# smolGura/fish-tts

Measured on AMD Instinct MI355X. Metric: semantic tokens/sec, higher is better.
Workload: dtype bf16; 1 GPU; openaudio-s1-mini shapes (BASELINE configs[1]): batch=1 per GPU, 48-token prompt, 215 frames (10 s), top-p sampling, hipGraph-captured frame step, + DAC codec decode; prompt_len=48, parallelism=replica x1, frame_engine=3

## Files before the change

fish-tts_amd/csrc/engine.hip:

```cpp
#include "engine.h"
#include "ar_kernels.h"
#include "frame_engine.h"
#include "wide_kernels.h"
#include "codec_kernels.h"

#include <math.h>

#include <algorithm>
#include <mutex>
#include <stdarg.h>
#include <stdio.h>
#include <stdlib.h>
#include <string.h>

using namespace ft;

static std::string g_create_err;
static void eng_release(ft_ctx* ctx);

ft_status ft_fail(ft_ctx* ctx, ft_status code, const std::string& msg) {
    if (ctx) ctx->err = msg; else g_create_err = msg;
    return code;
}

// ... 2051 lines not shown
            if (it->first & (1 << 28)) { hipGraphExecDestroy(it->second); it = ctx->graphs.erase(it); } else ++it;
        }
        eng_release(ctx);
        snprintf(buf, sizeof buf, "launch path: the frame engine was turned off after %d hand-off time-outs (last in phase %u)",
                 ctx->eng_strikes, w[ENG_CTL_WHERE]);
        ctx->eng_why = buf;
    }
    fprintf(stderr, "fish_tts_amd: frame engine: a hand-off timed out (phase %u, strike %d of %d): the frames are redone on the "
            "launch path%s\n", w[ENG_CTL_WHERE], ctx->eng_strikes, ENG_MAX_STRIKES,
            ctx->eng_strikes >= ENG_MAX_STRIKES ? "; the engine stays off for this context" : "");
    return FT_OK;
}
static bool eng_in_use(const ft_ctx* ctx) { return (ctx->eng_on || ctx->eng_fast_on) && !ctx->eng_suspended; }

extern "C" ft_status ft_ar_engine_state(ft_ctx* ctx, int32_t* flags, int32_t* aborted, int32_t* where) {
    FT_TRY(ar_ready(ctx));
    if (flags) *flags = (ctx->eng_on ? 1 : 0) | (ctx->eng_fast_on ? 2 : 0);
    if (aborted) *aborted = ctx->eng_strikes;
    if (where) *where = ctx->eng_last_where;
    return FT_OK;
}

extern "C" const char* ft_ar_frame_path(const ft_ctx* ctx) {
    if (!ctx) return "";
    ft_ctx* c = const_cast<ft_ctx*>(ctx);
    c->path_str = ctx->eng_why + (ctx->wide_ok
                                      ? "; lock-step batches of >= 5 rows: MFMA launches with fused row operations (five per layer)"
                                      : "; lock-step batches: multi-row GEMV launches");
    return c->path_str.c_str();
}

extern "C" ft_status ft_test_engine_fault(ft_ctx* ctx, int32_t which, int32_t wg, int32_t skip) {
    FT_TRY(ar_ready(ctx));
    if (!ctx->eng_ctl || !(which == 0 ? ctx->eng_on : ctx->eng_fast_on)) return ft_fail(ctx, FT_ERR_STATE, "ft_test_engine_fault: the frame engine is off");
    if (wg < 0 || wg >= ctx->eng_nb || skip < 0) return ft_fail(ctx, FT_ERR_ARG, "ft_test_engine_fault: bad workgroup or skip count");
    const unsigned v[2] = {(which == 0 ? 0u : ENG_FAULT_FAST) + 1u + (unsigned)wg, (unsigned)skip};
    static_assert(ENG_CTL_FAULT_SKIP == ENG_CTL_FAULT + 1, "the two words are written by one copy");
    FT_HIP(ctx, hipStreamSynchronize(ctx->stream));
    FT_HIP(ctx, hipMemcpy(ctx->eng_ctl + ENG_CTL_FAULT, v, sizeof v, hipMemcpyHostToDevice));
    return FT_OK;
}

extern "C" ft_status ft_test_ar_attn_plan(ft_ctx* ctx, int32_t* nsplit, int32_t* xl, int32_t* n_slots) {
    FT_TRY(ar_ready(ctx));
    if (nsplit) *nsplit = ctx->nsplit;
    if (xl) *xl = ctx->eng_on && ctx->eng_xl ? 1 : 0;
    if (n_slots) *n_slots = ctx->n_slots;
    return FT_OK;
}

namespace {
extern "C" ft_status ft_test_ar_trace_arm(ft_ctx* ctx, int32_t first, int32_t count) {
    FT_TRY(ar_ready(ctx));
    if (first < 0 || count < 0) return ft_fail(ctx, FT_ERR_ARG, "ft_test_ar_trace_arm: bad range");
    if (ctx->c.max_batch == 1 && eng_in_use(ctx))
        return ft_fail(ctx, FT_ERR_STATE, "ft_test_ar_trace_arm: this context's frames run on the frame engine");
    ArTrace& t = ctx->tstore;
    t.recs.clear();
    t.first = first; t.count = count; t.armed = true; t.failed = false; t.kind = 0;
    return FT_OK;
}
extern "C" int32_t ft_test_ar_trace_count(ft_ctx* ctx, int32_t* info) {
    if (!ctx || !ctx->has_ar) return -1;
    const ArTrace& t = ctx->tstore;
    if (info) { info[0] = t.kind; info[1] = t.m0; info[2] = t.M; info[3] = t.armed ? 1 : 0; info[4] = (int32_t)t.begin.size(); }
    return t.failed ? -1 : (int32_t)t.recs.size();
}
extern "C" ft_status ft_test_ar_trace_launch(ft_ctx* ctx, int32_t i, char* name, int32_t cap, int32_t* info) {
    if (!ctx || !ctx->has_ar || !name || cap < 1 || !info) return FT_ERR_ARG;
// ... 1148 lines not shown
```

fish-tts_amd/csrc/frame_engine.h:

```cpp
#pragma once
#include "ar_kernels.h"

namespace ft {

constexpr int ENG_NB = 256;
constexpr int ENG_WAVES = 8;
constexpr int ENG_THREADS = ENG_WAVES * 64;
constexpr int ENG_CW = 4;
constexpr int ENG_GW = 4;

template <int D_, int H_, int HKV_, int HDIM_, int F_>
struct EngSlowShape {
    static constexpr int D = D_, H = H_, HKV = HKV_, HDIM = HDIM_, F = F_;
    static constexpr int HD = H * HDIM, QKVN = (H + 2 * HKV) * HDIM, G = H / HKV;
    static constexpr int NTD = D / 512, NTA = HD / 512, NTF = F / 512;
    static constexpr int SQ = (QKVN / ENG_NB + ENG_CW - 1) / ENG_CW, SF = (F / ENG_NB + ENG_CW - 1) / ENG_CW, SO = (D / ENG_NB + ENG_CW - 1) / ENG_CW;
    static constexpr bool PK3 = F % 384 == 0 && (F / ENG_NB) % 3 == 0;
    static_assert(D % 512 == 0 && HD % 512 == 0 && F % 512 == 0, "weight rows are read as whole 16-byte pieces by 64 lanes");
    static_assert(QKVN % (4 * ENG_NB) == 0 && D % (4 * ENG_NB) == 0 && F % (4 * ENG_NB) == 0, "whole 16-byte granule groups per workgroup");
    static_assert(H % HKV == 0 && HDIM % 8 == 0 && HDIM <= 128, "grouped-query attention, 16-byte K/V pieces");
};
template <int D_, int H_, int HKV_, int HDIM_, int F_, int V_>
struct EngFastShape {
    static constexpr int D = D_, H = H_, HKV = HKV_, HDIM = HDIM_, F = F_, V = V_;
    static constexpr int HD = H * HDIM, QKVN = (H + 2 * HKV) * HDIM, KVW = HKV * HDIM;
    static constexpr int NTD = D / 512, NTA = HD / 512, NTF = F / 512;
    static constexpr int SQ = (QKVN / ENG_NB + ENG_CW - 1) / ENG_CW, SF = (F / ENG_NB + ENG_CW - 1) / ENG_CW, SO = (D / ENG_NB + ENG_CW - 1) / ENG_CW;
    static constexpr bool PK3 = F % 384 == 0 && (F / ENG_NB) % 3 == 0;
    static constexpr int RESF = (NTD <= 2 && F / ENG_NB == 12) ? 2 : 0;
    static constexpr int RESL = RESF ? 4 : 0;
    static_assert(D % 512 == 0 && HD % 512 == 0 && F % 512 == 0 && V == 1024 && HD == D, "fast widths");
    static_assert(QKVN % (4 * ENG_NB) == 0 && D % (4 * ENG_NB) == 0 && F % (4 * ENG_NB) == 0 && V % (4 * ENG_NB) == 0, "whole granule groups per workgroup");
};
typedef EngSlowShape<1024, 16, 8, 128, 3072> EngSlowS1;
typedef EngFastShape<1024, 16, 8, 64, 3072, 1024> EngFastS1;
constexpr int ENG_EPOCH_STEP = 64;
constexpr unsigned long long ENG_TIMEOUT_TICKS = 20000000ull;

typedef __attribute__((address_space(1))) unsigned eng_gu32;
typedef __attribute__((address_space(1))) unsigned long long eng_gu64;
#define ENG_RLX __ATOMIC_RELAXED, __HIP_MEMORY_SCOPE_AGENT

enum { ENG_CTL_EPOCH = 0, ENG_CTL_ABORT = 1, ENG_CTL_EXIT = 2, ENG_CTL_WHERE = 3, ENG_CTL_ARRIVED = 4, ENG_CTL_FAULT = 5, ENG_CTL_FAULT_SKIP = 6,
       ENG_CTL_XCD = 16, ENG_CTL_WORDS = 32 };
constexpr unsigned ENG_FAULT_FAST = 0x10000u;
__device__ __forceinline__ bool eng_fault_here(unsigned* ctl, unsigned base, int b) {
    const unsigned f = __hip_atomic_load((__attribute__((address_space(1))) unsigned*)(ctl + ENG_CTL_FAULT), __ATOMIC_RELAXED, __HIP_MEMORY_SCOPE_AGENT);
    if (f != base + 1u + (unsigned)b) return false;
    const unsigned skip = __hip_atomic_load((__attribute__((address_space(1))) unsigned*)(ctl + ENG_CTL_FAULT_SKIP), __ATOMIC_RELAXED, __HIP_MEMORY_SCOPE_AGENT);
    if (skip > 0u) {
        __hip_atomic_store((__attribute__((address_space(1))) unsigned*)(ctl + ENG_CTL_FAULT_SKIP), skip - 1u, __ATOMIC_RELAXED, __HIP_MEMORY_SCOPE_AGENT);
        return false;
    }
    __hip_atomic_store((__attribute__((address_space(1))) unsigned*)(ctl + ENG_CTL_FAULT), 0u, __ATOMIC_RELAXED, __HIP_MEMORY_SCOPE_AGENT);
    return true;
}

struct EngLayer {
    const bf16_t *wqkv, *bqkv, *attn_norm, *qn, *kn, *wo, *bo, *ffn_norm, *w13, *w2;
    bf16_t *kc, *vc;
};

__device__ __forceinline__ void eng_barrier() {
    __builtin_amdgcn_fence(__ATOMIC_RELEASE, "workgroup", "local");
    __builtin_amdgcn_s_barrier();
    __builtin_amdgcn_fence(__ATOMIC_ACQUIRE, "workgroup", "local");
}

typedef const __attribute__((address_space(1))) U4* eng_gU4;
template <bool NT> __device__ __forceinline__ U4 eng_ldg16(const void* p) {
    if constexpr (NT) return __builtin_nontemporal_load((eng_gU4)p);
    else return *(eng_gU4)p;
}
__device__ __forceinline__ float eng_ldg_bf16(const bf16_t* p, size_t i) {
    return bf16_bits_to_f32(((const __attribute__((address_space(1))) bf16_t*)p)[i]);
}
typedef const __attribute__((address_space(4))) unsigned long long* eng_c64;
__device__ __forceinline__ EngLayer eng_layer(const EngLayer* table, int i) {
    static_assert(sizeof(EngLayer) == 12 * sizeof(unsigned long long), "EngLayer is twelve pointers");
    eng_c64 q = (eng_c64)(unsigned long long)(table + i);
    EngLayer l;
    l.wqkv = (const bf16_t*)q[0]; l.bqkv = (const bf16_t*)q[1]; l.attn_norm = (const bf16_t*)q[2]; l.qn = (const bf16_t*)q[3];
    l.kn = (const bf16_t*)q[4]; l.wo = (const bf16_t*)q[5]; l.bo = (const bf16_t*)q[6]; l.ffn_norm = (const bf16_t*)q[7];
    l.w13 = (const bf16_t*)q[8]; l.w2 = (const bf16_t*)q[9]; l.kc = (bf16_t*)q[10]; l.vc = (bf16_t*)q[11];
    return l;
}

__device__ __forceinline__ unsigned eng_tag16(unsigned e) { return (e & 0x7fffu) | 0x8000u; }
// ... 76 lines not shown
    EngSpin sp{ctl, dead, 0, 0, where};
    unsigned long long n_full = 0, t_first = 0;
    for (int p0 = gw; p0 < npiece; p0 += 3 * ngw) {
        const int c0 = p0;
        const int c1 = p0 + ngw < npiece ? p0 + ngw : c0;
        const int c2 = p0 + 2 * ngw < npiece ? p0 + 2 * ngw : c0;
        const int i0 = c0 * 256 + lane * 4 < n ? c0 * 256 + lane * 4 : c0 * 256;
        const int i1 = c1 * 256 + lane * 4 < n ? c1 * 256 + lane * 4 : c1 * 256;
        const int i2 = c2 * 256 + lane * 4 < n ? c2 * 256 + lane * 4 : c2 * 256;
        const int o0 = lay.off(u0 + i0), o1 = lay.off(u0 + i1), o2 = lay.off(u0 + i2);
        U4 a, b, c;
        for (;;) {
            if (c1 == c0) { eng_ld1_sc1<FL>(g + o0, a); b = a; c = a; }
            else eng_ld3_sc1<FL>(g + o0, g + o1, g + o2, a, b, c);
            const bool oa = eng_tags_ok(a, tag), ob = eng_tags_ok(b, tag), oc = eng_tags_ok(c, tag);
            if (dbg && n_full == 0) t_first = eng_rt();
            ++n_full;
            if (__all(oa && ob && oc)) break;
            if (sp.give_up(lane)) return;
        }
        if (c0 * 256 + lane * 4 < n) eng_unpack_to_lds(dst + dmap(i0), a);
        if (c1 != c0 && c1 * 256 + lane * 4 < n) eng_unpack_to_lds(dst + dmap(i1), b);
        if (c2 != c0 && c2 * 256 + lane * 4 < n) eng_unpack_to_lds(dst + dmap(i2), c);
    }
    if (dbg && lane == 0) { dbg[0] = t_first; dbg[1] = n_full; dbg[2] = 0; }
}

struct EngRelay {
    int on;
    int rank, nr;
    long delta;
};

__device__ __forceinline__ void eng_register(unsigned* ctl, int nb, int* r, int* dead) {
    const int xcd = (int)(__builtin_amdgcn_s_getreg(20 | (0 << 6) | (3 << 11)) & 7u);
    const unsigned rank = atomicAdd(ctl + ENG_CTL_XCD + xcd, 1u);
    atomicAdd(ctl + ENG_CTL_ARRIVED, 1u);
    EngSpin sp{ctl, dead, 0, 0, 9999};
    bool ok = true;
    while (__hip_atomic_load((eng_gu32*)(ctl + ENG_CTL_ARRIVED), ENG_RLX) < (unsigned)nb) {
        if (sp.give_up(0)) { ok = false; break; }
        __builtin_amdgcn_s_sleep(2);
    }
    r[0] = xcd; r[1] = (int)rank;
    r[2] = ok ? (int)__hip_atomic_load((eng_gu32*)(ctl + ENG_CTL_XCD + xcd), ENG_RLX) : 1;
}

template <typename DMap = EngIdent>
__device__ __forceinline__ void eng_gather_x(const EngRelay& rl, const unsigned* g, EngLayout lay, int u0, int n, unsigned tag, float* dst,
                                             int gw, int ngw, int lane, unsigned* ctl, int* dead, int where, DMap dmap = DMap(),
                                             unsigned long long* dbg = nullptr) {
    if (!rl.on) { eng_gather(g, lay, u0, n, tag, dst, gw, ngw, lane, ctl, dead, where, dmap, dbg); return; }
    unsigned* rep = const_cast<unsigned*>(g) + rl.delta;
    const int npiece = (n + 255) >> 8;
    for (int p = rl.rank; p < npiece; p += rl.nr) {
        if (p % ngw != gw) continue;
        const int i = p * 256 + lane * 4 < n ? p * 256 + lane * 4 : p * 256;
        const int o = lay.off(u0 + i);
        EngSpin sp{ctl, dead, 0, 0, where};
        U4 a;
        for (;;) {
            eng_ld1_sc1(g + o, a);
            if (__all(eng_tags_ok(a, tag))) break;
            if (sp.give_up(lane)) return;
        }
        if (p * 256 + lane * 4 < n) *reinterpret_cast<U4*>(rep + o) = a;
    }
    eng_gather<DMap, 1>(rep, lay, u0, n, tag, dst, gw, ngw, lane, ctl, dead, where, dmap, dbg);
}

__device__ __forceinline__ bool eng_tags3_ok(const U4& v, unsigned tag) { return (v.y >> 16) == tag && (v.w >> 16) == tag; }
__device__ __forceinline__ void eng_unpack3_to_lds(float* dst, const U4& v) {
    float2 a, b, c;
    a.x = __uint_as_float(v.x << 16); a.y = __uint_as_float(v.x & 0xffff0000u);
    b.x = __uint_as_float(v.y << 16); b.y = __uint_as_float(v.z << 16);
    c.x = __uint_as_float(v.z & 0xffff0000u); c.y = __uint_as_float(v.w << 16);
    reinterpret_cast<float2*>(dst)[0] = a; reinterpret_cast<float2*>(dst)[1] = b; reinterpret_cast<float2*>(dst)[2] = c;
}
// ... 375 lines not shown
    eng_gemv2_part<NT, RPU, MAXS, PRO, EPI, ENG_CW>(r, xs0, xs1, K, eps, bias, resid0, resid1, gout0, gout1, tag0, tag1, u_lo, u_hi, u_lo, u_hi,
                                                    cw, lane, eo);
}

__device__ __forceinline__ void eng_units(int U, int b, int nb, int& lo, int& hi) {
    lo = (int)((long)U * b / nb);
    hi = (int)((long)U * (b + 1) / nb);
}

struct SlowEngP {
    const EngLayer* layers;
    int n_layer;
    int D, H, Hkv, hd, F, qkvN;
    float eps, scale;
    const bf16_t* emb; const bf16_t* cb_emb; const int* toks; long tok_row_stride;
    int ncb, cbsize, vocab, sem_begin, sem_end, scale_cb; float inv_div;
    const float* rope; const int* pos; int pos_off; int n_slots, nsplit;
    size_t cache_off;
    unsigned* gx;
    unsigned* gqkv;
    unsigned long long* gpart;
    unsigned* gy;
    unsigned* gxb;
    unsigned* gg;
    unsigned* ctl;
    long rep_delta0, rep_stride;
    float* x_out;
    int nt;
    unsigned long long* stamps;
};
#define ENG_STAMP(k) do { if (p.stamps && tid == 0) p.stamps[((size_t)b * p.n_layer + li) * 16 + (k)] = eng_rt(); } while (0)
#define ENG_ASTAMP(wv, k) do { if (p.stamps && gw == (wv) && lane == 0) \
    p.stamps[((size_t)nb * p.n_layer + (size_t)b * p.n_layer + li) * 16 + (k)] = eng_rt(); } while (0)

constexpr int ENG_KVST = 6;

__device__ __forceinline__ int eng_att_role(int b, int nb, int li, int natt) {
    int a = b - (int)(((unsigned)li * (unsigned)natt) % (unsigned)nb);
    if (a < 0) a += nb;
    return a < natt ? a : -1;
}

template <typename S, bool XL = false>
__global__ __launch_bounds__(ENG_THREADS) void slow_engine_kernel(SlowEngP p) {
    constexpr int NTD = S::NTD, NTA = S::NTA, NTF = S::NTF, G = S::G;
    constexpr int SQ = S::SQ, SF = S::SF, SO = S::SO;
    extern __shared__ __attribute__((aligned(16))) float smem[];
    const int tid = threadIdx.x, lane = tid & 63, wave = __builtin_amdgcn_readfirstlane(tid >> 6);
    const int b = blockIdx.x;
    constexpr int nb = ENG_NB;
    const int cw = wave;
    const int gw = wave - ENG_CW;
    const int atid = tid - ENG_CW * 64;
    constexpr int D = S::D, F = S::F, hd = S::HDIM, hp = hd >> 1, H = S::H, Hkv = S::HKV, HD = H * hd, QKVN = (H + 2 * Hkv) * hd;
    static_assert(!XL || (ENG_NB % Hkv == 0 && QKVN % ENG_NB == 0), "XCD-local attention: the workgroups of an XCD share one kv head's rows");
    float* xA = smem;
    float* yS = xA + D;
    float* xB = yS + HD;
    float* gS = xB + D;
    float* qS = gS + F;
    float* q_s = qS + (G + 2) * hd;
    float* k_new = q_s + G * hd;
    float* v_new = k_new + hd;
    constexpr int LPP = hd >> 3, PPW = 64 / LPP, NSLOT = 4 * PPW;
    float* ml_s = v_new + hd;
    float* acc_s = ml_s + NSLOT * G * 2;
    float* mscr = acc_s + NSLOT * G * hd;
    float* outS = mscr + 64 * 6;
    int* dead = reinterpret_cast<int*>(outS + ENG_MAX_OUT);
    int* out_count = dead + 1;
    int* reg_s = dead + 4;
    if (tid == 0) { *dead = eng_fault_here(p.ctl, 0u, b) ? 1 : 0; *out_count = 0; }
    if (tid == ENG_CW * 64) {
        reg_s[0] = 0; reg_s[1] = 0; reg_s[2] = 1;
        if (XL || p.rep_stride) eng_register(p.ctl, nb, reg_s, dead);
        if (XL && (reg_s[2] * Hkv != nb || reg_s[0] >= Hkv || reg_s[1] >= reg_s[2] || p.nsplit != reg_s[2])) {
            if (!__hip_atomic_load((eng_gu32*)(p.ctl + ENG_CTL_ABORT), ENG_RLX)) __hip_atomic_store((eng_gu32*)(p.ctl + ENG_CTL_WHERE), 9998u, ENG_RLX);
            __hip_atomic_store((eng_gu32*)(p.ctl + ENG_CTL_ABORT), 1u, ENG_RLX);
            reg_s[0] = 0; reg_s[1] = 0;
            *dead = 1;
        }
    }
    const unsigned epoch = __hip_atomic_load((eng_gu32*)(p.ctl + ENG_CTL_EPOCH), ENG_RLX);
    const int pos = p.pos[0] + p.pos_off;
    unsigned long long clk0 = 0, rt0 = 0;
    if (p.stamps) { clk0 = __builtin_amdgcn_s_memtime(); rt0 = eng_rt(); }
    const size_t VSTR = (size_t)nb * ENG_LINE;
    const EngLayout layD{D / nb}, layF{F / nb}, layQ{QKVN / nb}, layLin{0};
    const int nsplit = XL ? nb / Hkv : p.nsplit;
    const int natt = Hkv * nsplit;
    const int chunk = (pos + nsplit) / nsplit;
    const int grp = lane / LPP, gl = lane % LPP;

    {
        const int* tk = p.toks;
        int t0 = tk[0];
        const bool is_vq = t0 >= p.sem_begin && t0 <= p.sem_end;
        t0 = min(max(t0, 0), p.vocab - 1);
        for (int d = tid; d < D; d += ENG_THREADS) {
            float vq = 0.f;
            if (is_vq) {
                constexpr int MAXCB = 16;
                for (int i0 = 0; i0 < p.ncb; i0 += MAXCB) {
                    int c[MAXCB];
                    float e[MAXCB];
#pragma unroll
                    for (int i = 0; i < MAXCB; ++i) c[i] = i0 + i < p.ncb ? tk[(size_t)(i0 + i + 1) * p.tok_row_stride] : 0;
#pragma unroll
                    for (int i = 0; i < MAXCB; ++i) {
                        const int cc = min(max(c[i], 0), p.cbsize - 1);
                        e[i] = i0 + i < p.ncb ? ld_elem(p.cb_emb, (size_t)(cc + (i0 + i) * p.cbsize) * D + d) : 0.f;
// ... 9 lines not shown
        }
    }

    if (wave < ENG_CW) {
        int q_lo, q_hi, o_lo, o_hi, f_lo, f_hi, d_lo, d_hi;
        eng_units(QKVN, b, nb, q_lo, q_hi);
        if (XL) { q_lo = 0; q_hi = QKVN / nb; }
        eng_units(D, b, nb, o_lo, o_hi);
        eng_units(F, b, nb, f_lo, f_hi);
        eng_units(D, b, nb, d_lo, d_hi);
        EngW<NTD, 1, SQ> wq;
        EngW<NTA, 1, SO> wo;
        EngW<NTD, 2, SF> wf;
        EngW<NTF, 1, SO> wd;
        EngOut eo{outS, out_count, 0};
        {
            const EngLayer l0 = eng_layer(p.layers, 0);
            if (!XL) eng_issue(wq, l0.wqkv, l0.attn_norm, D, q_lo, q_hi, cw, lane, p.nt);
            eng_issue(wo, l0.wo, (const bf16_t*)nullptr, HD, o_lo, o_hi, cw, lane, p.nt);
            eng_issue(wf, l0.w13, l0.ffn_norm, D, f_lo, f_hi, cw, lane, p.nt);
            eng_issue(wd, l0.w2, (const bf16_t*)nullptr, F, d_lo, d_hi, cw, lane, p.nt);
            __builtin_amdgcn_sched_barrier(0);
        }
        eng_barrier();
        const int xnq = G * hd * Hkv / nb, xnk = hd * Hkv / nb;
        const EngRowQkvX rmq{reg_s[0] * G * hd + reg_s[1] * xnq, (H + reg_s[0]) * hd + reg_s[1] * xnk,
                             (H + Hkv + reg_s[0]) * hd + reg_s[1] * xnk, xnq, xnk};
        if (XL) {
            const EngLayer l0 = eng_layer(p.layers, 0);
            eng_issue(wq, l0.wqkv, l0.attn_norm, D, q_lo, q_hi, cw, lane, p.nt, rmq);
            __builtin_amdgcn_sched_barrier(0);
        }
        eng_barrier();
        for (int li = 0; li < p.n_layer; ++li) {
            const int par = li & 1, parn = (li + 1) & 1;
            const unsigned tag = eng_tag16(epoch + (unsigned)li);
            const unsigned tagn = eng_tag16(epoch + (unsigned)li + 1u);
            const EngLayer l = eng_layer(p.layers, li);
            const bool more = li + 1 < p.n_layer;
            const EngLayer ln = eng_layer(p.layers, more ? li + 1 : li);
            if (li > 0) { eng_barrier(); if (*dead) break; }
            ENG_STAMP(0);
            if (XL)
                eng_gemv_qkv_local<NTD, SQ>(wq, xA, D, p.eps, l.bqkv, p.gqkv + (size_t)par * VSTR, tag, q_hi, cw, lane, eo, rmq);
            else
                eng_gemv<NTD, 1, SQ, PRO_RMSNORM, EPI_STORE>(wq, xA, D, p.eps, l.bqkv, nullptr, p.gqkv + (size_t)par * VSTR + eng_pub(b, q_lo), tag, nullptr,
                                                             q_lo, q_hi, cw, lane, eo);
            __builtin_amdgcn_sched_barrier(0);
            ENG_STAMP(1);
            if (more) {
                if (XL) eng_issue(wq, ln.wqkv, ln.attn_norm, D, q_lo, q_hi, cw, lane, p.nt, rmq);
                else eng_issue(wq, ln.wqkv, ln.attn_norm, D, q_lo, q_hi, cw, lane, p.nt);
            }
            __builtin_amdgcn_sched_barrier(0);
            if (XL || eng_att_role(b, nb, li, natt) >= 0) {
                eng_barrier(); if (*dead) break;
                eng_barrier();
                eng_barrier();
            }
            ENG_STAMP(2);
            eng_barrier(); if (*dead) break;
            ENG_STAMP(3);
            eng_gemv<NTA, 1, SO, PRO_NONE, EPI_RESID>(wo, yS, HD, p.eps, l.bo, xA, p.gxb + (size_t)par * VSTR + eng_pub(b, o_lo), tag, nullptr, o_lo, o_hi, cw, lane, eo);
            __builtin_amdgcn_sched_barrier(0);
            ENG_STAMP(4);
            if (p.stamps && (p.nt & 2)) { asm volatile("s_waitcnt vmcnt(0)" ::: "memory"); ENG_STAMP(9); }
// ... 379 lines not shown
                                ENG_MSTEP(1) ENG_MSTEP(2) ENG_MSTEP(3) ENG_MSTEP(4) ENG_MSTEP(5) ENG_MSTEP(6) ENG_MSTEP(7)
#undef ENG_MSTEP
                            }
                        }
                        if (alive && s8 == 0 && item_on) {
                            unsigned* gy = p.gy + (size_t)par * HD + (size_t)a * (G * epb) + g * epb + (e - split * epb);
                            eng_put4(gy, round_bf16(a0 / L), round_bf16(a1 / L), round_bf16(a2 / L), round_bf16(a3 / L), tag);
                        }
                    }
                    ENG_ASTAMP(3, 6);
                }
            }
            {
                const int epb = hd / nsplit, ns = nsplit;
                auto ymap = [=](int i) { const int a2 = i / (G * epb), r2 = i % (G * epb), g2 = r2 / epb, eo = r2 % epb;
                                         return ((a2 / ns) * G + g2) * hd + (a2 % ns) * epb + eo; };
                eng_gather_x(rl, p.gy + (size_t)par * HD, layLin, 0, HD, tag, yS, gw, ENG_GW, lane, p.ctl, dead, li * 8 + 3, ymap);
            }
            eng_barrier(); if (*dead) break;
            if (a >= 0) kv_issue();
            const unsigned long long t_poll0 = p.stamps ? eng_rt() : 0ull;
            eng_gather_x(rl, p.gxb + (size_t)par * VSTR, layD, 0, D, tag, xB, gw, ENG_GW, lane, p.ctl, dead, li * 8 + 4, EngIdent(),
                       (p.stamps && gw == 0) ? p.stamps + ((size_t)b * p.n_layer + li) * 16 + 13 : nullptr);
            const unsigned long long t_poll1 = p.stamps ? eng_rt() : 0ull;
            eng_barrier(); if (*dead) break;
            if (p.stamps && tid == ENG_CW * 64) {
                unsigned long long* q = p.stamps + ((size_t)b * p.n_layer + li) * 16;
                q[10] = t_poll0; q[11] = t_poll1; q[12] = eng_rt();
            }
            if constexpr (S::PK3) eng_gather3_x(rl, p.gg + (size_t)par * VSTR, F, tag, gS, gw, ENG_GW, lane, p.ctl, dead, li * 8 + 5);
            else eng_gather_x(rl, p.gg + (size_t)par * VSTR, layF, 0, F, tag, gS, gw, ENG_GW, lane, p.ctl, dead, li * 8 + 5);
            eng_barrier(); if (*dead) break;
        }
    }

    eng_barrier();
    if (p.stamps && tid == 0 && b == 0) {
        p.stamps[14] = __builtin_amdgcn_s_memtime() - clk0; p.stamps[15] = eng_rt() - rt0;
    }
    if (tid == 0) {
        const unsigned old = atomicAdd(p.ctl + ENG_CTL_EXIT, 1u);
        if (old + 1 == (unsigned)nb) {
            __hip_atomic_store((eng_gu32*)(p.ctl + ENG_CTL_EXIT), 0u, ENG_RLX);
            __hip_atomic_store((eng_gu32*)(p.ctl + ENG_CTL_ARRIVED), 0u, ENG_RLX);
            for (int x = 0; x < 8; ++x) __hip_atomic_store((eng_gu32*)(p.ctl + ENG_CTL_XCD + x), 0u, ENG_RLX);
            __hip_atomic_store((eng_gu32*)(p.ctl + ENG_CTL_EPOCH), epoch + ENG_EPOCH_STEP, ENG_RLX);
        }
    }
}

struct FastEngP {
    const EngLayer* layers;
    int n_layer, ncb;
    int D, H, Hkv, hd, F, qkvN, V;
    float eps, scale;
    const float* rope;
    const bf16_t* fast_norm; const bf16_t* fast_out; const bf16_t* fast_emb;
    const float* hid;
    const float* femb;
    unsigned* gx;
    unsigned* gqkv;
    unsigned* gxb;
    unsigned* gg;
    unsigned* glog;
    unsigned* gcode;
    unsigned* ctl;
    long rep_delta0, rep_stride;
    SampP samp;
    long noise_cb_stride;
    long noise_off1;
    int pair;
    const bf16_t* qkv0_tab;
    unsigned long long* stamps;
    int nt;
};
#define ENG_FSTAMP(k) do { if (p.stamps && tid == 0) p.stamps[(((size_t)b * p.ncb + cb) * nL + li) * 16 + (k)] = eng_rt(); } while (0)

#define ENG_GSTAMP(k) do { if (p.stamps && atid == 0) p.stamps[(((size_t)b * p.ncb + cb) * nL + nL - 1) * 16 + (k)] = eng_rt(); } while (0)
constexpr int ENG_FV = 1024;

struct EngSub {
    int* end_at;
    int n;
    __device__ __forceinline__ void sync(int) { ++n; eng_barrier(); }
};
__device__ __forceinline__ void eng_draw_follow(const int* end_at) {
    for (int c = 1;; ++c) {
        eng_barrier();
        if (*reinterpret_cast<const volatile int*>(end_at) == c) break;
    }
}

template <int MAXCB, int HD>
__device__ __forceinline__ void eng_fast_attn(const float* qkvS, bf16_t* kS, bf16_t* vS, float* yS, const bf16_t* qn, const bf16_t* kn,
                                              const float (&cs)[2], const float (&sn)[2], int c, int ncb, int H, int Hkv, float eps, float scale,
                                              int w, int nw, int lane) {
    constexpr int EPL = HD > 64 ? 2 : 1;
    const int G = H / Hkv;
    for (int h = w; h < H; h += nw) {
        const int kvh = h / G;
        bf16_t* kh = kS + (size_t)kvh * ncb * HD + lane;
        bf16_t* vh = vS + (size_t)kvh * ncb * HD + lane;
        const float* qp = qkvS + h * HD + lane;
        const float* kp = qkvS + (H + kvh) * HD + lane;
        const float* vp = qkvS + (H + Hkv + kvh) * HD + lane;
        float q[EPL], kx[EPL], vx[EPL];
#pragma unroll
        for (int e = 0; e < EPL; ++e) { q[e] = qp[64 * e]; kx[e] = kp[64 * e]; vx[e] = vp[64 * e]; }
        if (c == 0) {
// ... 507 lines not shown
    constexpr int D = FS::D, F = FS::F, hd = HDIM, H = FS::H, Hkv = FS::HKV, HD = H * hd, KVW = Hkv * hd, QKVN = (H + 2 * Hkv) * hd, V = FS::V;
    float* xA = smem;
    float* qkvS = xA + D;
    float* yS = qkvS + QKVN;
    float* xB = yS + HD;
    float* gS = xB + D;
    float* logS = gS + F;
    float* outS = logS + V;
    float* redbuf = outS + ENG_MAX_OUT;
    int* pen_id = reinterpret_cast<int*>(redbuf + 8);
    float* pen_val = reinterpret_cast<float*>(pen_id + 32);
    float* amv = pen_val + 32;
    int* ami = reinterpret_cast<int*>(amv + 8);
    int* wcnt = ami + 8;
    float* prL = reinterpret_cast<float*>(wcnt + 4);
    uint32_t* keyL = reinterpret_cast<uint32_t*>(prL + 1024);
    uint32_t* cut = keyL + 1024;
    int* dead = reinterpret_cast<int*>(cut + 4);
    int* out_count = dead + 1;
    int* sub_count = dead + 2;
    int* codes_s = dead + 4;
    int* reg_s = codes_s + MAXCB;
    bf16_t* kvS = reinterpret_cast<bf16_t*>(reg_s + 4);
    float* xA1 = smem + ((((size_t)(reinterpret_cast<float*>(kvS + (size_t)p.n_layer * 2 * p.ncb * KVW) - smem)) + 3) & ~(size_t)3);
    float* xB1 = xA1 + D;
    float* gS1 = xB1 + D;
    float* qkvS1 = gS1;
    float* yS1 = gS1 + QKVN;
    int f_lo, f_hi;
    eng_units(F, b, nb, f_lo, f_hi);
    const int f_c_hi = f_hi - FRES;
    EngW<NTD, 2, (RF ? RF : 1)> res[RL ? RL : 1];
    if (p.stamps && tid == 0) p.stamps[(size_t)b * p.ncb * p.n_layer * 16 + 15] = eng_rt();
    if (tid == 0) { *dead = eng_fault_here(p.ctl, ENG_FAULT_FAST, b) ? 1 : 0; *out_count = 0; *sub_count = 0; dead[3] = 0; }
    if (tid == ENG_CW * 64) {
        reg_s[0] = 0; reg_s[1] = 0; reg_s[2] = 1;
        if (p.rep_stride) eng_register(p.ctl, nb, reg_s, dead);
    }
    const unsigned epoch = __hip_atomic_load((eng_gu32*)(p.ctl + ENG_CTL_EPOCH), ENG_RLX);
    const size_t VSTR = (size_t)nb * ENG_LINE;
    const EngLayout layD{D / nb}, layF{F / nb}, layQ{QKVN / nb}, layV{V / nb};
    const int nL = p.n_layer;
    auto bx = [&](int par, int l) { return p.gx + ((size_t)par * (nL + 1) + l) * VSTR; };
    auto bq = [&](int par, int l) { return p.gqkv + ((size_t)par * nL + l) * VSTR; };
    auto bxb = [&](int par, int l) { return p.gxb + ((size_t)par * nL + l) * VSTR; };
    auto bg = [&](int par, int l) { return p.gg + ((size_t)par * nL + l) * VSTR; };
    auto blog = [&](int par) { return p.glog + (size_t)par * VSTR; };
    auto drawer = [&](int cb) { return (cb * 37) % nb; };
    bool alive = true;
    const bool pair = p.pair != 0 && p.ncb >= 2;

    if (wave < ENG_CW) {
        int q_lo, q_hi, o_lo, o_hi, h_lo, h_hi;
        eng_units(QKVN, b, nb, q_lo, q_hi);
        eng_units(D, b, nb, o_lo, o_hi);
        eng_units(V, b, nb, h_lo, h_hi);
        EngW<NTD, 1, SQ> wq;
        EngW<NTA, 1, SO> wo;
        EngW<NTD, 2, SFC> wf;
        EngW<NTF, 1, SO> wd;
        EngW<NTD, 1, SO> wh;
        EngOut eo{outS, out_count, 0};
        EngOut eo13{outS, dead + 3, 0};
        EngOut& eoF = RES ? eo13 : eo;
        {
            const EngLayer l0 = eng_layer(p.layers, 0);
            eng_issue<false>(wq, l0.wqkv, l0.attn_norm, D, q_lo, q_hi, cw, lane, p.nt);
            eng_issue<false>(wo, l0.wo, (const bf16_t*)nullptr, HD, o_lo, o_hi, cw, lane, p.nt);
            eng_issue<false>(wf, l0.w13, l0.ffn_norm, D, f_lo, f_c_hi, cw, lane, p.nt);
            eng_issue<false>(wd, l0.w2, (const bf16_t*)nullptr, F, o_lo, o_hi, cw, lane, p.nt);
// ... 341 lines not shown
                    if (*reinterpret_cast<volatile int*>(sub_count) == 0) {
                        const int last = cb == p.ncb - 1;
                        const int nfv = pre.nfv;
                        EngSampLds S{redbuf, pen_id, pen_val, amv, ami, wcnt, prL, keyL, cut};
                        const int code = eng_sample_small(sp, pre, logS, S, sub, at, dl, gw,
                                                          p.stamps ? p.stamps + (((size_t)b * p.ncb + cb) * nL + nL - 1) * 16 : nullptr);
                        ENG_GSTAMP(14);
                        const int R = p.ncb + 1;
                        if (atid == 0) { codes_s[cb] = code; *sub_count = sub.n + 1; }
                        sub.sync(lane);
                        prev_code = code;
                        if (b == drawer(cb)) {
                            if (atid == 0) sp.tokn[cb + 1] = code;
                            if (last) {
                                const int frozen = sp.done[0];
                                if (atid < R) {
                                    const int v = atid < 2 ? sp.tokn[atid] : (atid - 1 == cb ? code : codes_s[atid - 1]);
                                    sp.tok[atid] = v;
                                    if (nfv < sp.cap && !frozen) sp.seq[(size_t)atid * sp.cap + nfv] = v;
                                }
                                if (atid == 0 && !frozen) {
                                    sp.pos[0] += 1;
                                    sp.nf[0] = nfv + 1;
                                    if (sp.tokn[0] == sp.im_end) sp.done[0] = 1;
                                }
                            }
                        }
                    }
                }
            }
        }
    }

    eng_barrier();
    if (tid == 0) {
        const unsigned old = atomicAdd(p.ctl + ENG_CTL_EXIT, 1u);
        if (old + 1 == (unsigned)nb) {
            __hip_atomic_store((eng_gu32*)(p.ctl + ENG_CTL_EXIT), 0u, ENG_RLX);
            __hip_atomic_store((eng_gu32*)(p.ctl + ENG_CTL_ARRIVED), 0u, ENG_RLX);
            for (int x = 0; x < 8; ++x) __hip_atomic_store((eng_gu32*)(p.ctl + ENG_CTL_XCD + x), 0u, ENG_RLX);
            __hip_atomic_store((eng_gu32*)(p.ctl + ENG_CTL_EPOCH), epoch + ENG_EPOCH_STEP, ENG_RLX);
        }
    }
}

}
```

Measured before the change: 787.4 tokens/s.

## Replace grid-wide arrival spin and exit counter with per-XCD census settled by one workgroup

Workgroup registration no longer spins until every workgroup has arrived on a shared counter. Each workgroup takes a rank from a per-XCD counter, and each counter now sits on its own cache line. The end-of-kernel exit counter is removed: workgroup 0 checks the census, resets the counters and advances the epoch, while the other workgroups return early unless stamps are enabled. The goal is to cut startup and teardown synchronisation in the persistent frame engine. In exchange it assumes an even XCD distribution and now detects imbalance only at the end, and it adds fault-injection kinds for testing.

```diff
diff --git a/fish-tts_amd/csrc/engine.hip b/fish-tts_amd/csrc/engine.hip
--- a/fish-tts_amd/csrc/engine.hip
+++ b/fish-tts_amd/csrc/engine.hip
@@ -2107,9 +2107,12 @@
 
 extern "C" ft_status ft_test_engine_fault(ft_ctx* ctx, int32_t which, int32_t wg, int32_t skip) {
     FT_TRY(ar_ready(ctx));
-    if (!ctx->eng_ctl || !(which == 0 ? ctx->eng_on : ctx->eng_fast_on)) return ft_fail(ctx, FT_ERR_STATE, "ft_test_engine_fault: the frame engine is off");
+    if (which < 0 || which > 5) return ft_fail(ctx, FT_ERR_ARG, "ft_test_engine_fault: which is 0..5");
+    const bool fast = (which & 1) != 0;
+    if (!ctx->eng_ctl || !(fast ? ctx->eng_fast_on : ctx->eng_on)) return ft_fail(ctx, FT_ERR_STATE, "ft_test_engine_fault: the frame engine is off");
     if (wg < 0 || wg >= ctx->eng_nb || skip < 0) return ft_fail(ctx, FT_ERR_ARG, "ft_test_engine_fault: bad workgroup or skip count");
-    const unsigned v[2] = {(which == 0 ? 0u : ENG_FAULT_FAST) + 1u + (unsigned)wg, (unsigned)skip};
+    const unsigned kind = which >> 1 == 1 ? ENG_FAULT_RANK : which >> 1 == 2 ? ENG_FAULT_MARK : 0u;
+    const unsigned v[2] = {(fast ? ENG_FAULT_FAST : 0u) + kind + 1u + (unsigned)wg, (unsigned)skip};
     static_assert(ENG_CTL_FAULT_SKIP == ENG_CTL_FAULT + 1, "the two words are written by one copy");
     FT_HIP(ctx, hipStreamSynchronize(ctx->stream));
     FT_HIP(ctx, hipMemcpy(ctx->eng_ctl + ENG_CTL_FAULT, v, sizeof v, hipMemcpyHostToDevice));
diff --git a/fish-tts_amd/csrc/frame_engine.h b/fish-tts_amd/csrc/frame_engine.h
--- a/fish-tts_amd/csrc/frame_engine.h
+++ b/fish-tts_amd/csrc/frame_engine.h
@@ -41,19 +41,22 @@
 typedef __attribute__((address_space(1))) unsigned long long eng_gu64;
 #define ENG_RLX __ATOMIC_RELAXED, __HIP_MEMORY_SCOPE_AGENT
 
-enum { ENG_CTL_EPOCH = 0, ENG_CTL_ABORT = 1, ENG_CTL_EXIT = 2, ENG_CTL_WHERE = 3, ENG_CTL_ARRIVED = 4, ENG_CTL_FAULT = 5, ENG_CTL_FAULT_SKIP = 6,
-       ENG_CTL_XCD = 16, ENG_CTL_WORDS = 32 };
-constexpr unsigned ENG_FAULT_FAST = 0x10000u;
-__device__ __forceinline__ bool eng_fault_here(unsigned* ctl, unsigned base, int b) {
+constexpr int ENG_CTL_LINE = 32;
+enum { ENG_CTL_EPOCH = 0, ENG_CTL_ABORT = 1, ENG_CTL_WHERE = 3, ENG_CTL_FAULT = 5, ENG_CTL_FAULT_SKIP = 6,
+       ENG_CTL_XCD = ENG_CTL_LINE, ENG_CTL_WORDS = 9 * ENG_CTL_LINE };
+constexpr unsigned ENG_WHERE_CENSUS = 9998u;
+constexpr unsigned ENG_FAULT_FAST = 0x10000u, ENG_FAULT_RANK = 0x20000u, ENG_FAULT_MARK = 0x40000u;
+enum { ENG_FAULT_NONE = 0, ENG_FAULT_KIND_DEAD = 1, ENG_FAULT_KIND_RANK = 2, ENG_FAULT_KIND_MARK = 3 };
+__device__ __forceinline__ int eng_fault_here(unsigned* ctl, unsigned base, int b) {
     const unsigned f = __hip_atomic_load((__attribute__((address_space(1))) unsigned*)(ctl + ENG_CTL_FAULT), __ATOMIC_RELAXED, __HIP_MEMORY_SCOPE_AGENT);
-    if (f != base + 1u + (unsigned)b) return false;
+    if ((f & ~(ENG_FAULT_RANK | ENG_FAULT_MARK)) != base + 1u + (unsigned)b) return ENG_FAULT_NONE;
     const unsigned skip = __hip_atomic_load((__attribute__((address_space(1))) unsigned*)(ctl + ENG_CTL_FAULT_SKIP), __ATOMIC_RELAXED, __HIP_MEMORY_SCOPE_AGENT);
     if (skip > 0u) {
         __hip_atomic_store((__attribute__((address_space(1))) unsigned*)(ctl + ENG_CTL_FAULT_SKIP), skip - 1u, __ATOMIC_RELAXED, __HIP_MEMORY_SCOPE_AGENT);
-        return false;
+        return ENG_FAULT_NONE;
     }
     __hip_atomic_store((__attribute__((address_space(1))) unsigned*)(ctl + ENG_CTL_FAULT), 0u, __ATOMIC_RELAXED, __HIP_MEMORY_SCOPE_AGENT);
-    return true;
+    return (f & ENG_FAULT_RANK) ? ENG_FAULT_KIND_RANK : (f & ENG_FAULT_MARK) ? ENG_FAULT_KIND_MARK : ENG_FAULT_KIND_DEAD;
 }
 
 struct EngLayer {
@@ -196,18 +199,31 @@
     long delta;
 };
 
-__device__ __forceinline__ void eng_register(unsigned* ctl, int nb, int* r, int* dead) {
-    const int xcd = (int)(__builtin_amdgcn_s_getreg(20 | (0 << 6) | (3 << 11)) & 7u);
-    const unsigned rank = atomicAdd(ctl + ENG_CTL_XCD + xcd, 1u);
-    atomicAdd(ctl + ENG_CTL_ARRIVED, 1u);
-    EngSpin sp{ctl, dead, 0, 0, 9999};
-    bool ok = true;
-    while (__hip_atomic_load((eng_gu32*)(ctl + ENG_CTL_ARRIVED), ENG_RLX) < (unsigned)nb) {
-        if (sp.give_up(0)) { ok = false; break; }
-        __builtin_amdgcn_s_sleep(2);
-    }
-    r[0] = xcd; r[1] = (int)rank;
-    r[2] = ok ? (int)__hip_atomic_load((eng_gu32*)(ctl + ENG_CTL_XCD + xcd), ENG_RLX) : 1;
+__device__ __forceinline__ int eng_xcd() { return (int)(__builtin_amdgcn_s_getreg(20 | (0 << 6) | (3 << 11)) & 7u); }
+__device__ __forceinline__ void eng_raise(unsigned* ctl, unsigned where) {
+    if (!__hip_atomic_load((eng_gu32*)(ctl + ENG_CTL_ABORT), ENG_RLX)) __hip_atomic_store((eng_gu32*)(ctl + ENG_CTL_WHERE), where, ENG_RLX);
+    __hip_atomic_store((eng_gu32*)(ctl + ENG_CTL_ABORT), 1u, ENG_RLX);
+}
+__device__ __forceinline__ void eng_register(unsigned* ctl, unsigned fault_base, int b, bool reg, int* r, int* dead) {
+    const int xcd = eng_xcd();
+    unsigned rank = 0u;
+    if (reg) rank = atomicAdd(ctl + ENG_CTL_XCD + xcd * ENG_CTL_LINE, 1u);
+    const int fault = eng_fault_here(ctl, fault_base, b);
+    if (reg && fault == ENG_FAULT_KIND_MARK) atomicAdd(ctl + ENG_CTL_XCD + ((xcd + 1) & 7) * ENG_CTL_LINE, 1u);
+    const bool ok = !reg || (rank < (unsigned)(ENG_NB / 8) && fault != ENG_FAULT_KIND_RANK);
+    r[0] = reg ? xcd : 0; r[1] = ok ? (int)rank : 0; r[2] = reg ? ENG_NB / 8 : 1;
+    if (!ok) eng_raise(ctl, ENG_WHERE_CENSUS);
+    *dead = (!ok || fault == ENG_FAULT_KIND_DEAD) ? 1 : 0;
+}
+__device__ __forceinline__ void eng_settle(unsigned* ctl, bool registered, int lane) {
+    const int w = lane < 8 ? ENG_CTL_XCD + lane * ENG_CTL_LINE : ENG_CTL_EPOCH;
+    unsigned n = (unsigned)(ENG_NB / 8);
+    if (lane <= 8) {
+        n = __hip_atomic_load((eng_gu32*)(ctl + w), ENG_RLX);
+        __hip_atomic_store((eng_gu32*)(ctl + w), lane < 8 ? 0u : n + (unsigned)ENG_EPOCH_STEP, ENG_RLX);
+    }
+    const bool even = __all(lane >= 8 || n == (unsigned)(ENG_NB / 8));
+    if (lane == 0 && registered && !even) eng_raise(ctl, ENG_WHERE_CENSUS);
 }
 
 template <typename DMap = EngIdent>
@@ -649,6 +665,8 @@
 #define ENG_STAMP(k) do { if (p.stamps && tid == 0) p.stamps[((size_t)b * p.n_layer + li) * 16 + (k)] = eng_rt(); } while (0)
 #define ENG_ASTAMP(wv, k) do { if (p.stamps && gw == (wv) && lane == 0) \
     p.stamps[((size_t)nb * p.n_layer + (size_t)b * p.n_layer + li) * 16 + (k)] = eng_rt(); } while (0)
+
+#define ENG_HSTAMP(k) do { if (p.stamps) p.stamps[((size_t)nb * p.n_layer + (size_t)b * p.n_layer) * 16 + (k)] = eng_rt(); } while (0)
 
 constexpr int ENG_KVST = 6;
 
@@ -687,13 +705,13 @@
     int* dead = reinterpret_cast<int*>(outS + ENG_MAX_OUT);
     int* out_count = dead + 1;
     int* reg_s = dead + 4;
-    if (tid == 0) { *dead = eng_fault_here(p.ctl, 0u, b) ? 1 : 0; *out_count = 0; }
+    if (tid == 0) { ENG_HSTAMP(9); *out_count = 0; }
     if (tid == ENG_CW * 64) {
-        reg_s[0] = 0; reg_s[1] = 0; reg_s[2] = 1;
-        if (XL || p.rep_stride) eng_register(p.ctl, nb, reg_s, dead);
-        if (XL && (reg_s[2] * Hkv != nb || reg_s[0] >= Hkv || reg_s[1] >= reg_s[2] || p.nsplit != reg_s[2])) {
-            if (!__hip_atomic_load((eng_gu32*)(p.ctl + ENG_CTL_ABORT), ENG_RLX)) __hip_atomic_store((eng_gu32*)(p.ctl + ENG_CTL_WHERE), 9998u, ENG_RLX);
-            __hip_atomic_store((eng_gu32*)(p.ctl + ENG_CTL_ABORT), 1u, ENG_RLX);
+        eng_register(p.ctl, 0u, b, !(p.nt & 4) && (XL || p.rep_stride), reg_s, dead);
+        if (p.nt & 4) { reg_s[0] = eng_xcd(); reg_s[1] = b >> 3; reg_s[2] = nb / 8; }
+        ENG_HSTAMP(10);
+        if (XL && (reg_s[2] * Hkv != nb || reg_s[0] >= Hkv || p.nsplit != reg_s[2])) {
+            eng_raise(p.ctl, ENG_WHERE_CENSUS);
             reg_s[0] = 0; reg_s[1] = 0;
             *dead = 1;
         }
@@ -769,6 +787,7 @@
             __builtin_amdgcn_sched_barrier(0);
         }
         eng_barrier();
+        if (tid == 0) ENG_HSTAMP(11);
         for (int li = 0; li < p.n_layer; ++li) {
             const int par = li & 1, parn = (li + 1) & 1;
             const unsigned tag = eng_tag16(epoch + (unsigned)li);
@@ -1214,21 +1233,16 @@
             else eng_gather_x(rl, p.gg + (size_t)par * VSTR, layF, 0, F, tag, gS, gw, ENG_GW, lane, p.ctl, dead, li * 8 + 5);
             eng_barrier(); if (*dead) break;
         }
-    }
-
+        if (b == 0 && gw == 0 && !*dead && !(p.nt & 4)) eng_settle(p.ctl, XL || p.rep_stride != 0, lane);
+    }
+
+    if (!p.stamps) return;
     eng_barrier();
     if (p.stamps && tid == 0 && b == 0) {
         p.stamps[14] = __builtin_amdgcn_s_memtime() - clk0; p.stamps[15] = eng_rt() - rt0;
     }
-    if (tid == 0) {
-        const unsigned old = atomicAdd(p.ctl + ENG_CTL_EXIT, 1u);
-        if (old + 1 == (unsigned)nb) {
-            __hip_atomic_store((eng_gu32*)(p.ctl + ENG_CTL_EXIT), 0u, ENG_RLX);
-            __hip_atomic_store((eng_gu32*)(p.ctl + ENG_CTL_ARRIVED), 0u, ENG_RLX);
-            for (int x = 0; x < 8; ++x) __hip_atomic_store((eng_gu32*)(p.ctl + ENG_CTL_XCD + x), 0u, ENG_RLX);
-            __hip_atomic_store((eng_gu32*)(p.ctl + ENG_CTL_EPOCH), epoch + ENG_EPOCH_STEP, ENG_RLX);
-        }
-    }
+    if (tid == 0) ENG_HSTAMP(12);
+    if (tid == 0 && p.stamps) { asm volatile("s_waitcnt vmcnt(0)" ::: "memory"); ENG_HSTAMP(13); }
 }
 
 struct FastEngP {
@@ -1257,6 +1271,7 @@
     int nt;
 };
 #define ENG_FSTAMP(k) do { if (p.stamps && tid == 0) p.stamps[(((size_t)b * p.ncb + cb) * nL + li) * 16 + (k)] = eng_rt(); } while (0)
+#define ENG_FHSTAMP(k) do { if (p.stamps) p.stamps[(size_t)b * p.ncb * p.n_layer * 16 + (k)] = eng_rt(); } while (0)
 
 #define ENG_GSTAMP(k) do { if (p.stamps && atid == 0) p.stamps[(((size_t)b * p.ncb + cb) * nL + nL - 1) * 16 + (k)] = eng_rt(); } while (0)
 constexpr int ENG_FV = 1024;
@@ -1830,10 +1845,11 @@
     const int f_c_hi = f_hi - FRES;
     EngW<NTD, 2, (RF ? RF : 1)> res[RL ? RL : 1];
     if (p.stamps && tid == 0) p.stamps[(size_t)b * p.ncb * p.n_layer * 16 + 15] = eng_rt();
-    if (tid == 0) { *dead = eng_fault_here(p.ctl, ENG_FAULT_FAST, b) ? 1 : 0; *out_count = 0; *sub_count = 0; dead[3] = 0; }
+    if (tid == 0) { *out_count = 0; *sub_count = 0; dead[3] = 0; }
     if (tid == ENG_CW * 64) {
-        reg_s[0] = 0; reg_s[1] = 0; reg_s[2] = 1;
-        if (p.rep_stride) eng_register(p.ctl, nb, reg_s, dead);
+        eng_register(p.ctl, ENG_FAULT_FAST, b, !(p.nt & 4) && p.rep_stride != 0, reg_s, dead);
+        if (p.nt & 4) { reg_s[0] = eng_xcd(); reg_s[1] = b >> 3; reg_s[2] = nb / 8; }
+        ENG_FHSTAMP(13);
     }
     const unsigned epoch = __hip_atomic_load((eng_gu32*)(p.ctl + ENG_CTL_EPOCH), ENG_RLX);
     const size_t VSTR = (size_t)nb * ENG_LINE;
@@ -2241,16 +2257,11 @@
         }
     }
 
+    if (alive && !*dead && b == 0 && wave == 0 && !(p.nt & 4)) eng_settle(p.ctl, p.rep_stride != 0, lane);
+    if (!p.stamps) return;
     eng_barrier();
-    if (tid == 0) {
-        const unsigned old = atomicAdd(p.ctl + ENG_CTL_EXIT, 1u);
-        if (old + 1 == (unsigned)nb) {
-            __hip_atomic_store((eng_gu32*)(p.ctl + ENG_CTL_EXIT), 0u, ENG_RLX);
-            __hip_atomic_store((eng_gu32*)(p.ctl + ENG_CTL_ARRIVED), 0u, ENG_RLX);
-            for (int x = 0; x < 8; ++x) __hip_atomic_store((eng_gu32*)(p.ctl + ENG_CTL_XCD + x), 0u, ENG_RLX);
-            __hip_atomic_store((eng_gu32*)(p.ctl + ENG_CTL_EPOCH), epoch + ENG_EPOCH_STEP, ENG_RLX);
-        }
-    }
-}
-
-}
+    if (tid == 0) ENG_FHSTAMP(12);
+    if (tid == 0 && p.stamps) { asm volatile("s_waitcnt vmcnt(0)" ::: "memory"); ENG_FHSTAMP(11); }
+}
+
+}
```

After: 794.9 tokens/s, median of 6. About the same (+1.0%).
